# JiahaoPlus/EvoWorld

Measured on AMD Instinct MI355X. Metric: panoramic frames/sec per clip (576x1024x25f, 25 denoise steps), higher is better.
Workload: dtype f16

## Files before the change

evoworld_amd/csrc/norm.hip:

```cpp
#include "common.h"
#include <cstdlib>

namespace {

inline int gn_chunks(int n_slabs, int rows) {
    constexpr int target = 640;
    int want = (target + n_slabs - 1) / n_slabs;
    const int cap = (rows + 63) / 64;
    if (want > cap) want = cap;
    if (want > 512) want = 512;
    return want < 1 ? 1 : want;
}

__global__ void gn_stats_kernel(const f16* __restrict__ x, const int8_t* __restrict__ x_lo, float* __restrict__ part,
                                float* __restrict__ pivot, int rows, int C_src, int c_off, int C_tot, int VPP, int PL,
                                int rows_per_block) {
    extern __shared__ float lds[];
    const int tid = threadIdx.x;
    const int slab = blockIdx.y;
    const int v = tid % VPP, pl = tid / VPP;
    const int r0 = blockIdx.x * rows_per_block;
    const int r1 = min(rows, r0 + rows_per_block);
    float s[8], q[8], piv[8];
    const size_t slab_off = ((size_t)slab * rows) * C_src + v * 8;
// ... 60 lines not shown
                const float f = (float)val[e] - piv[e];
                s[e] += f;
                q[e] += f * f;
            }
        }
    }
    float* mine = lds + (size_t)pl * 2 * C_src;
#pragma unroll
    for (int e = 0; e < 8; ++e) {
        mine[v * 8 + e] = s[e];
        mine[C_src + v * 8 + e] = q[e];
    }
    __syncthreads();
    float* dst = part + (((size_t)slab * gridDim.x + blockIdx.x) * C_tot + c_off) * 2;
    for (int c = tid; c < C_src; c += blockDim.x) {
        float ss = 0.f, qq = 0.f;
        for (int k = 0; k < PL; ++k) { ss += lds[(size_t)k * 2 * C_src + c]; qq += lds[(size_t)k * 2 * C_src + C_src + c]; }
        *(f32x2*)(dst + 2 * c) = (f32x2){ss, qq};
    }
    if (blockIdx.x == 0 && pl == 0) {
#pragma unroll
        for (int e = 0; e < 8; ++e) pivot[(size_t)slab * C_tot + c_off + v * 8 + e] = piv[e];
    }
}

__global__ __launch_bounds__(256) void gn_finalize_kernel(const float* __restrict__ part, const float* __restrict__ pivot,
                                                          float* __restrict__ stats, int n_slabs, int rows, int C_tot,
                                                          int groups, int chunks) {
    __shared__ float red[2][256];
    __shared__ float chan[2][512];
    __shared__ float wsum[4];
    const int tid = threadIdx.x;
    const int slab = blockIdx.x / groups, g = blockIdx.x - slab * groups;
    const int gs = C_tot / groups;
    const float n = (float)rows;
    const int cw = gs < 256 ? gs : 256;
    const int KP = 256 / cw;
    for (int c0 = 0; c0 < gs; c0 += cw) {
        const int c = c0 + tid % cw, kc = tid / cw;
        float ss = 0.f, qq = 0.f;
        if (kc < KP && c < gs) {
            const float* p = part + (((size_t)slab * chunks) * C_tot + g * gs + c) * 2;
            for (int k = kc; k < chunks; k += KP) {
                const f32x2 v = *(const f32x2*)(p + (size_t)k * C_tot * 2);
                ss += v[0];
                qq += v[1];
            }
        }
        red[0][tid] = ss;
        red[1][tid] = qq;
        __syncthreads();
        if (tid < cw && c0 + tid < gs) {
            float s2 = 0.f, q2 = 0.f;
            for (int k = 0; k < KP; ++k) { s2 += red[0][k * cw + tid]; q2 += red[1][k * cw + tid]; }
            const float d = s2 / n;
            chan[0][c0 + tid] = pivot[(size_t)slab * C_tot + g * gs + c0 + tid] + d;
            chan[1][c0 + tid] = fmaxf(q2 - s2 * d, 0.f);
        }
        __syncthreads();
    }
    float ms = 0.f, m2 = 0.f;
    for (int c = tid; c < gs; c += 256) { ms += chan[0][c]; m2 += chan[1][c]; }
    ms = wave_sum(ms);
    m2 = wave_sum(m2);
    if ((tid & 63) == 0) wsum[tid >> 6] = ms;
    __syncthreads();
    const float mean = (wsum[0] + wsum[1] + wsum[2] + wsum[3]) / (float)gs;
    __syncthreads();
    float dev = 0.f;
    for (int c = tid; c < gs; c += 256) { const float d = chan[0][c] - mean; dev += d * d; }
    dev = wave_sum(dev);
    if ((tid & 63) == 0) { wsum[tid >> 6] = m2 + n * dev; }
    __syncthreads();
    if (tid == 0) *(f32x2*)(stats + (size_t)blockIdx.x * 2) = (f32x2){mean, (wsum[0] + wsum[1] + wsum[2] + wsum[3]) / (n * (float)gs)};
}

template <bool LO, bool YLO>
__global__ void gn_apply_kernel(const f16* __restrict__ x, const int8_t* __restrict__ x_lo, const float* __restrict__ stats,
                                const f16* __restrict__ gamma, const f16* __restrict__ beta, f16* __restrict__ y,
                                f16* __restrict__ y_lo, int ld_y, int rows,
                                int C_src, int c_off, int C_tot, int groups, float eps, int silu, int VPP, int PL,
                                int rows_per_block) {
    const int tid = threadIdx.x;
    const int slab = blockIdx.y;
    const int v = tid % VPP, pl = tid / VPP;
    const int c = v * 8;
    const int gs = C_tot / groups;
    const f16x8 gm = *(const f16x8*)(gamma + c_off + c);
    const f16x8 bt = *(const f16x8*)(beta + c_off + c);
    float scale[8], shift[8];
    int gprev = -1;
    float mean = 0.f, rstd = 0.f;
#pragma unroll
    for (int e = 0; e < 8; ++e) {
        const int g = (c_off + c + e) / gs;
        if (g != gprev) {
            gprev = g;
            const f32x2 st = *(const f32x2*)(stats + ((size_t)slab * groups + g) * 2);
            mean = st[0];
            rstd = rsqrtf(st[1] + eps);
        }
        scale[e] = rstd;
        shift[e] = mean;
    }
    const int r0 = blockIdx.x * rows_per_block;
    const int r1 = min(rows, r0 + rows_per_block);
    const f16* xin = x + ((size_t)slab * rows) * C_src + c;
    const int8_t* xlo = LO ? x_lo + ((size_t)slab * rows) * C_src + c : nullptr;
    f16* yout = y + ((size_t)slab * rows) * ld_y + c_off + c;
    f16* ylo = YLO ? y_lo + ((size_t)slab * rows) * ld_y + c_off + c : nullptr;
    int r = r0 + pl;
    for (; r + 3 * PL < r1; r += 4 * PL) {
        f16x8 val[4];
        u32x2 vlo[4];
#pragma unroll
        for (int u = 0; u < 4; ++u) {
            val[u] = *(const f16x8*)(xin + (size_t)(r + u * PL) * C_src);
            if constexpr (LO) vlo[u] = *(const u32x2*)(xlo + (size_t)(r + u * PL) * C_src);
        }
#pragma unroll
        for (int u = 0; u < 4; ++u) {
            f16x8 o, ol;
#pragma unroll
            for (int e = 0; e < 8; ++e) {
                float xv;
                if constexpr (LO) xv = ew_split_dec(val[u][e], ew_sbyte(vlo[u][e >> 2], e & 3));
                else xv = (float)val[u][e];
                float f = (xv - shift[e]) * scale[e] * (float)gm[e] + (float)bt[e];
                if (silu) f = ew_silu(f);
                o[e] = (f16)f;
                if constexpr (YLO) ol[e] = (f16)(f - (float)o[e]);
            }
            *(f16x8*)(yout + (size_t)(r + u * PL) * ld_y) = o;
            if constexpr (YLO) *(f16x8*)(ylo + (size_t)(r + u * PL) * ld_y) = ol;
        }
    }
    for (; r < r1; r += PL) {
        const f16x8 val = *(const f16x8*)(xin + (size_t)r * C_src);
        u32x2 vlo;
        if constexpr (LO) vlo = *(const u32x2*)(xlo + (size_t)r * C_src);
        f16x8 o, ol;
#pragma unroll
        for (int e = 0; e < 8; ++e) {
            float xv;
            if constexpr (LO) xv = ew_split_dec(val[e], ew_sbyte(vlo[e >> 2], e & 3));
            else xv = (float)val[e];
            float f = (xv - shift[e]) * scale[e] * (float)gm[e] + (float)bt[e];
            if (silu) f = ew_silu(f);
            o[e] = (f16)f;
            if constexpr (YLO) ol[e] = (f16)(f - (float)o[e]);
        }
        *(f16x8*)(yout + (size_t)r * ld_y) = o;
        if constexpr (YLO) *(f16x8*)(ylo + (size_t)r * ld_y) = ol;
    }
}

template <int NV, int RPW>
__global__ __launch_bounds__(256) void ln_kernel(const f16* __restrict__ x, const int8_t* __restrict__ x_lo,
                                                 const f16* __restrict__ addvec, int rpg, f16* __restrict__ x_out,
                                                 int8_t* __restrict__ x_out_lo, const f16* __restrict__ gamma,
                                                 const f16* __restrict__ beta, f16* __restrict__ y, int rows, int C,
                                                 float eps) {
    const int lane = threadIdx.x & 63;
    const int row0 = (blockIdx.x * 4 + (threadIdx.x >> 6)) * RPW;
    if (row0 >= rows) return;
    const int VPP = C / 8;
    float v[RPW][NV][8];
    f16x8 raw[RPW][NV], add[RPW][NV];
    u32x2 rlo[RPW][NV];
#pragma unroll
    for (int r = 0; r < RPW; ++r) {
        const int row = min(row0 + r, rows - 1);
#pragma unroll
        for (int k = 0; k < NV; ++k) {
            const int vi = lane + k * 64;
            if (vi < VPP) {
                raw[r][k] = *(const f16x8*)(x + (size_t)row * C + vi * 8);
                if (x_lo) rlo[r][k] = *(const u32x2*)(x_lo + (size_t)row * C + vi * 8);
                if (addvec) add[r][k] = *(const f16x8*)(addvec + (size_t)(row / rpg) * C + vi * 8);
            }
        }
    }
    f16x8 g[NV], bta[NV];
#pragma unroll
    for (int k = 0; k < NV; ++k) {
        const int vi = lane + k * 64;
        if (vi < VPP) { g[k] = *(const f16x8*)(gamma + vi * 8); bta[k] = *(const f16x8*)(beta + vi * 8); }
    }
#pragma unroll
    for (int r = 0; r < RPW; ++r) {
        const int row = row0 + r;
        const bool live = row < rows;
        float sum = 0.f;
#pragma unroll
        for (int k = 0; k < NV; ++k) {
            const int vi = lane + k * 64;
            if (vi < VPP) {
                if (x_lo) {
                    ew_split_dec8(raw[r][k], rlo[r][k], v[r][k]);
                } else {
#pragma unroll
                    for (int e = 0; e < 8; ++e) v[r][k][e] = (float)raw[r][k][e];
                }
                if (addvec) {
                    f16x8 xo;
                    int s8[8];
#pragma unroll
                    for (int e = 0; e < 8; ++e) {
                        const float sum = v[r][k][e] + (float)add[r][k][e];
                        xo[e] = (f16)sum;
                        s8[e] = ew_split_enc(sum, xo[e]);
                        v[r][k][e] = !x_out ? sum : (x_out_lo ? ew_split_dec(xo[e], s8[e]) : (float)xo[e]);
                    }
                    if (x_out && live) *(f16x8*)(x_out + (size_t)row * C + vi * 8) = xo;
                    if (x_out_lo && live)
                        *(u32x2*)(x_out_lo + (size_t)row * C + vi * 8) =
                            (u32x2){ew_pack4(s8[0], s8[1], s8[2], s8[3]), ew_pack4(s8[4], s8[5], s8[6], s8[7])};
                }
#pragma unroll
                for (int e = 0; e < 8; ++e) sum += v[r][k][e];
            } else {
#pragma unroll
                for (int e = 0; e < 8; ++e) v[r][k][e] = 0.f;
            }
        }
        const float mean = wave_sum(sum) / (float)C;
        float sq = 0.f;
#pragma unroll
        for (int k = 0; k < NV; ++k) {
            const int vi = lane + k * 64;
            if (vi < VPP) {
#pragma unroll
                for (int e = 0; e < 8; ++e) { const float d = v[r][k][e] - mean; sq += d * d; }
            }
        }
        const float rstd = rsqrtf(wave_sum(sq) / (float)C + eps);
#pragma unroll
        for (int k = 0; k < NV; ++k) {
            const int vi = lane + k * 64;
            if (vi < VPP && live) {
                f16x8 o;
#pragma unroll
                for (int e = 0; e < 8; ++e) o[e] = (f16)((v[r][k][e] - mean) * rstd * (float)g[k][e] + (float)bta[k][e]);
                *(f16x8*)(y + (size_t)row * C + vi * 8) = o;
            }
        }
    }
}

}

extern "C" size_t ew_groupnorm_workspace_floats(int n_slabs, int rows, int C_tot, int groups) {
    if (n_slabs <= 0 || rows <= 0 || C_tot <= 0 || groups <= 0) return 0;
    return (size_t)n_slabs * gn_chunks(n_slabs, rows) * C_tot * 2 + (size_t)n_slabs * C_tot + (size_t)n_slabs * groups * 2;
}

namespace {
struct GnWs { float* part; float* pivot; float* stats; int chunks; };
inline GnWs gn_ws(float* ws, int n_slabs, int rows, int C_tot) {
    GnWs w;
    w.chunks = gn_chunks(n_slabs, rows);
    w.part = ws;
    w.pivot = ws + (size_t)n_slabs * w.chunks * C_tot * 2;
    w.stats = w.pivot + (size_t)n_slabs * C_tot;
    return w;
}
}

extern "C" ew_status ew_groupnorm_stats_f16(const void* x, const void* x_lo, float* ws, int n_slabs, int rows, int C_src,
                                            int c_off, int C_tot, int groups, void* stream) {
    EW_REQUIRE(x && ws, "ew_groupnorm_stats_f16: null pointer");
    EW_REQUIRE(n_slabs > 0 && rows > 0 && C_src > 0 && C_src % 8 == 0 && C_src <= 8192, "ew_groupnorm_stats_f16: bad shape");
    EW_REQUIRE(groups > 0 && C_tot % groups == 0 && c_off >= 0 && c_off + C_src <= C_tot, "ew_groupnorm_stats_f16: bad groups");
    const int VPP = C_src / 8;
    EW_REQUIRE(VPP <= 1024, "ew_groupnorm_stats_f16: C_src too large");
    const int PL = VPP >= 256 ? 1 : 256 / VPP;
    const GnWs w = gn_ws(ws, n_slabs, rows, C_tot);
    const int rpb = ew_cdiv(rows, w.chunks);
    dim3 grid(w.chunks, n_slabs);
    const size_t lds = (size_t)PL * 2 * C_src * sizeof(float);
    EW_REQUIRE(lds <= 64 * 1024, "ew_groupnorm_stats_f16: C_src too large for the LDS combine");
    hipLaunchKernelGGL(gn_stats_kernel, grid, dim3(VPP * PL), lds, (hipStream_t)stream, (const f16*)x, (const int8_t*)x_lo,
                       w.part, w.pivot, rows, C_src, c_off, C_tot, VPP, PL, rpb);
    return ew_check_launch("ew_groupnorm_stats_f16");
}

extern "C" ew_status ew_groupnorm_finalize(float* ws, int n_slabs, int rows, int C_tot, int groups, void* stream) {
    EW_REQUIRE(ws, "ew_groupnorm_finalize: null pointer");
    EW_REQUIRE(n_slabs > 0 && rows > 0 && groups > 0 && C_tot % groups == 0 && C_tot / groups <= 512,
               "ew_groupnorm_finalize: bad shape");
    const GnWs w = gn_ws(ws, n_slabs, rows, C_tot);
    hipLaunchKernelGGL(gn_finalize_kernel, dim3(n_slabs * groups), dim3(256), 0, (hipStream_t)stream,
                       w.part, w.pivot, w.stats, n_slabs, rows, C_tot, groups, w.chunks);
    return ew_check_launch("ew_groupnorm_finalize");
}

static ew_status gn_apply_launch(const char* what, const void* x, const void* x_lo, const float* ws, const void* gamma,
                                 const void* beta, void* y, void* y_lo, int ld_y, int n_slabs, int rows, int C_src, int c_off,
                                 int C_tot, int groups, float eps, int silu, void* stream) {
    EW_REQUIRE(x && ws && gamma && beta && y, "ew_groupnorm_apply: null pointer");
    EW_REQUIRE(n_slabs > 0 && rows > 0 && C_src > 0 && C_src % 8 == 0 && c_off % 8 == 0 && C_tot % 8 == 0,
               "ew_groupnorm_apply: bad shape");
    EW_REQUIRE(groups > 0 && C_tot % groups == 0 && c_off >= 0 && c_off + C_src <= C_tot, "ew_groupnorm_apply: bad groups");
    EW_REQUIRE(ld_y >= C_tot && ld_y % 8 == 0, "ew_groupnorm_apply: bad output row stride");
    const int VPP = C_src / 8;
    EW_REQUIRE(VPP <= 1024, "ew_groupnorm_apply: C_src too large");
    const int PL = VPP >= 256 ? 1 : 256 / VPP;
    const int rpb = 8 * PL;
    const GnWs w = gn_ws((float*)ws, n_slabs, rows, C_tot);
    dim3 grid(ew_cdiv(rows, rpb), n_slabs);
#define GN_APPLY(LO_, YLO_)                                                                                                      \
    hipLaunchKernelGGL((gn_apply_kernel<LO_, YLO_>), grid, dim3(VPP * PL), 0, (hipStream_t)stream, (const f16*)x,                  \
                       (const int8_t*)x_lo, w.stats, (const f16*)gamma, (const f16*)beta, (f16*)y, (f16*)y_lo, ld_y, rows, C_src,  \
                       c_off, C_tot, groups, eps, silu, VPP, PL, rpb)
    if (x_lo) { if (y_lo) GN_APPLY(true, true); else GN_APPLY(true, false); }
    else      { if (y_lo) GN_APPLY(false, true); else GN_APPLY(false, false); }
#undef GN_APPLY
    return ew_check_launch(what);
}

extern "C" ew_status ew_groupnorm_apply_f16(const void* x, const void* x_lo, const float* ws, const void* gamma,
                                            const void* beta, void* y, int n_slabs, int rows, int C_src, int c_off, int C_tot,
                                            int groups, float eps, int silu, void* stream) {
    return gn_apply_launch("ew_groupnorm_apply_f16", x, x_lo, ws, gamma, beta, y, nullptr, C_tot, n_slabs, rows, C_src, c_off, C_tot,
                           groups, eps, silu, stream);
}

extern "C" ew_status ew_groupnorm_apply_split_f16(const void* x, const void* x_lo, const float* ws, const void* gamma,
                                                  const void* beta, void* y, void* y_lo, int ld_y, int n_slabs, int rows, int C_src,
                                                  int c_off, int C_tot, int groups, float eps, int silu, void* stream) {
    EW_REQUIRE(y_lo, "ew_groupnorm_apply_split_f16: null pointer");
    return gn_apply_launch("ew_groupnorm_apply_split_f16", x, x_lo, ws, gamma, beta, y, y_lo, ld_y, n_slabs, rows, C_src, c_off, C_tot,
                           groups, eps, silu, stream);
}

extern "C" ew_status ew_layernorm_f16(const void* x, const void* x_lo, const void* addvec, int rows_per_group, void* x_out,
                                      void* x_out_lo, const void* gamma, const void* beta, void* y, int rows, int C, float eps,
                                      void* stream) {
    EW_REQUIRE(x && gamma && beta && y, "ew_layernorm_f16: null pointer");
    EW_REQUIRE(rows > 0 && C > 0 && C % 8 == 0 && C <= 2048, "ew_layernorm_f16: need C %% 8 == 0 and C <= 2048 (C=%d)", C);
    EW_REQUIRE(!addvec || rows_per_group >= 1, "ew_layernorm_f16: rows_per_group must be >= 1");
    EW_REQUIRE(!x_out_lo || (addvec && x_out), "ew_layernorm_f16: x_out_lo needs addvec and x_out");
    const int nv = (C / 8 + 63) / 64;
    dim3 block(256);
    hipStream_t s = (hipStream_t)stream;
    const int rpg = rows_per_group >= 1 ? rows_per_group : 1;
#define LN_LAUNCH(NV, RPW)                                                                                         \
    hipLaunchKernelGGL((ln_kernel<NV, RPW>), dim3(ew_cdiv(rows, 4 * RPW)), block, 0, s, (const f16*)x, (const int8_t*)x_lo, \
                       (const f16*)addvec, rpg, (f16*)x_out, (int8_t*)x_out_lo, (const f16*)gamma, (const f16*)beta, (f16*)y, rows, C, eps)
    if (nv == 1) LN_LAUNCH(1, 4);
    else if (nv == 2) LN_LAUNCH(2, 4);
    else if (nv == 3) LN_LAUNCH(3, 2);
    else LN_LAUNCH(4, 2);
#undef LN_LAUNCH
    return ew_check_launch("ew_layernorm_f16");
}
```

evoworld_amd/ops.py:

```python
import ctypes

import numpy as np
import torch

from . import _lib
from ._lib import GemmArgs

A_DENSE, A_CONV3X3, A_CONVT3 = _lib.EW_A_DENSE, _lib.EW_A_CONV3X3, _lib.EW_A_CONVT3
ACT_NONE, ACT_SILU, ACT_GEGLU, ACT_GELU = _lib.EW_ACT_NONE, _lib.EW_ACT_SILU, _lib.EW_ACT_GEGLU, _lib.EW_ACT_GELU

_zero_pages = {}


def _stream():
    return ctypes.c_void_p(torch.cuda.current_stream().cuda_stream)


def _ptr(t):
    return None if t is None else ctypes.c_void_p(t.data_ptr())


def _call(name, *args):
    _lib.check(getattr(_lib.load(), name)(*args, _stream()), name)


def _aligned(t, n=16):
    t = t.contiguous()
    return t if t.data_ptr() % n == 0 else t.clone(memory_format=torch.contiguous_format)


def _req(t, dtype, name):
    if t.device.type != "cuda":
        raise _lib.EvoWorldHipError(f"{name} must live on the GPU (got {t.device}); evoworld_amd has no CPU path")
    if t.dtype != dtype:
        raise TypeError(f"{name}: expected {dtype}, got {t.dtype}")
    if not t.is_contiguous():
        raise ValueError(f"{name} must be contiguous")
    return t


def zero_page(device):
    key = str(device)
    if key not in _zero_pages:
        _zero_pages[key] = torch.zeros(4096, dtype=torch.float16, device=device)
    return _zero_pages[key]


class Res:
    __slots__ = ("hi", "lo")

    def __init__(self, hi, lo=None):
        self.hi, self.lo = hi, lo

    @classmethod
    def empty(cls, rows, C, device, split):
        hi = torch.empty(rows, C, dtype=torch.float16, device=device)
        return cls(hi, torch.empty(rows, C, dtype=torch.int8, device=device) if split else None)

    @classmethod
    def from_float(cls, x):
        x = x.float().contiguous()
        hi = x.half()
        d = (x.view(torch.int32) - hi.float().view(torch.int32) + 16) >> 5
        return cls(hi, d.clamp_(-128, 127).to(torch.int8))

    def float(self):
        if self.lo is None:
            return self.hi.float()
        return (self.hi.float().contiguous().view(torch.int32) + (self.lo.to(torch.int32) << 5)).view(torch.float32)


def _hl(x):
    if x is None:
        return None, None
    if isinstance(x, Res):
        return x.hi, x.lo
    return x, None


def gemm(a, w, out, *, M, N, c1, lda, a2=None, c2=0, lda2=0, bias=None, rowbias=None, rows_per_group=1, ld_rowbias=None,
         r1=None, ld_r1=0, r2=None, ld_r2=0, ld_out=None, mode=A_DENSE, conv=None, tconv=None, act=ACT_NONE,
         c_acc=1.0, c_r1=1.0, c_r2=1.0, conv_shift=0):
    g = GemmArgs()
    r1h, r1l = _hl(r1)
    r2h, r2l = _hl(r2)
    outh, outl = _hl(out)
    g.a, g.a2, g.w, g.bias, g.rowbias = _ptr(a), _ptr(a2), _ptr(w), _ptr(bias), _ptr(rowbias)
    g.r1, g.r2, g.out, g.zero_page = _ptr(r1h), _ptr(r2h), _ptr(outh), _ptr(zero_page(a.device))
    g.r1_lo, g.r2_lo, g.out_lo = _ptr(r1l), _ptr(r2l), _ptr(outl)
    g.M, g.N, g.c1, g.c2, g.lda, g.lda2 = M, N, c1, c2, lda, lda2
    n_out = N // 2 if act == ACT_GEGLU else N
    g.ld_out = ld_out if ld_out is not None else n_out
    g.ld_r1, g.ld_r2, g.mode = ld_r1, ld_r2, mode
    g.ld_rowbias = ld_rowbias if ld_rowbias is not None else N
    if conv is not None:
        g.n_img, g.h_in, g.w_in, g.h_out, g.w_out, g.stride, g.upsample = conv
    if tconv is not None:
        g.tB, g.tT, g.tP = tconv
    g.rows_per_group, g.act = rows_per_group, act
    g.c_acc, g.c_r1, g.c_r2 = c_acc, c_r1, c_r2
    g.conv_shift = conv_shift
    _call("ew_gemm_f16", ctypes.byref(g))
    return out


_sk_ready = set()


def streamk_init():
    key = (torch.cuda.current_device(), torch.cuda.current_stream().cuda_stream)
    if key in _sk_ready:
        return
    if _lib.load().ew_get_gemm_generation() != 3:
        return
    if torch.cuda.is_current_stream_capturing():
        return
    _sk_ready.add(key)
    if _lib.load().ew_gemm_streamk_init(_stream()) != 0:
        import warnings
        msg = _lib.load().ew_last_error()
        warnings.warn("ew_gemm_streamk_init: " + (msg.decode() if msg else "failed") + " (continuing without the stream-K tail on this stream)")


def streamk_check():
    st = _lib.load().ew_gemm_streamk_status()
    if st != 0:
        msg = _lib.load().ew_last_error()
        raise _lib.EvoWorldHipError((msg.decode() if msg else "stream-K hand-over timed out in ew_gemm_f16 (generation 3): results of that launch are invalid")
                                    if st > 0 else "ew_gemm_streamk_status: HIP error while reading the status word")


def linear(x, w, bias=None, out=None, split_out=False, **kw):
    _req(x, torch.float16, "x"); _req(w, torch.float16, "w")
    M, K = x.shape
    N = w.shape[0]
    act = kw.get("act", ACT_NONE)
    if out is None:
        n_out = N // 2 if act == ACT_GEGLU else N
        out = Res.empty(M, n_out, x.device, True) if split_out else torch.empty(M, n_out, dtype=torch.float16, device=x.device)
    return gemm(x, w, out, M=M, N=N, c1=K, lda=K, bias=bias, **kw)


class WorkspacePool:

    def __init__(self, device, floats=8 << 20):
        self.buf = torch.empty(floats, dtype=torch.float32, device=device)
        self.cur = 0

    def reset(self):
        self.cur = 0

    def take(self, n):
        n = (n + 63) // 64 * 64
        if self.cur + n > self.buf.numel():
            return torch.empty(n, dtype=torch.float32, device=self.buf.device)
        v = self.buf[self.cur: self.cur + n]
        self.cur += n
        return v


def groupnorm(xs, gamma, beta, n_slabs, rows, eps, silu, groups=32, out=None, pool=None, stats_hi_only=False, split_out=False):
    lib = _lib.load()
    srcs = [_hl(x) for x in xs]
    C_tot = sum(h.shape[-1] for h, _ in srcs)
    dev = srcs[0][0].device
    nws = lib.ew_groupnorm_workspace_floats(n_slabs, rows, C_tot, groups)
    ws = pool.take(nws) if pool is not None else torch.empty(nws, dtype=torch.float32, device=dev)
    if out is None:
        out = torch.empty(n_slabs * rows, 2 * C_tot if split_out else C_tot, dtype=torch.float16, device=dev)
    off = 0
    for h, l in srcs:
        _call("ew_groupnorm_stats_f16", _ptr(h), None if stats_hi_only else _ptr(l), _ptr(ws), n_slabs, rows, h.shape[-1], off, C_tot, groups)
        off += h.shape[-1]
    _call("ew_groupnorm_finalize", _ptr(ws), n_slabs, rows, C_tot, groups)
    off = 0
    for h, l in srcs:
        if split_out:
            _call("ew_groupnorm_apply_split_f16", _ptr(h), _ptr(l), _ptr(ws), _ptr(gamma), _ptr(beta), _ptr(out), _ptr(out[:, C_tot:]),
                  2 * C_tot, n_slabs, rows, h.shape[-1], off, C_tot, groups, eps, 1 if silu else 0)
        else:
            _call("ew_groupnorm_apply_f16", _ptr(h), _ptr(l), _ptr(ws), _ptr(gamma), _ptr(beta), _ptr(out), n_slabs, rows,
                  h.shape[-1], off, C_tot, groups, eps, 1 if silu else 0)
        off += h.shape[-1]
    return out


def layernorm(x, gamma, beta, eps=1e-5, addvec=None, rows_per_group=1, x_out=None, out=None):
    xh, xl = _hl(x)
    oh, ol = _hl(x_out)
    rows, C = xh.shape
    if out is None:
        out = torch.empty_like(xh)
    _call("ew_layernorm_f16", _ptr(xh), _ptr(xl), _ptr(addvec), rows_per_group, _ptr(oh), _ptr(ol), _ptr(gamma), _ptr(beta), _ptr(out), rows, C, eps)
    return out


def attn_spatial(q, k, vt, o, n_seq, S, heads, ld_qk, ld_vt, ld_o, scale=0.125):
    _call("ew_attn_spatial_f16", _ptr(q), _ptr(k), _ptr(vt), _ptr(o), n_seq, S, heads, ld_qk, ld_vt, ld_o, scale)
    return o


QK_LOG2_PRESCALE = (0.125 * 1.4426950408889634) ** 0.5


def attn_spatial_log2(q, k, vt, o, n_seq, S, heads, ld_qk, ld_vt, ld_o):
    _call("ew_attn_spatial_log2_f16", _ptr(q), _ptr(k), _ptr(vt), _ptr(o), n_seq, S, heads, ld_qk, ld_vt, ld_o)
    return o


def quant_rows_fp8(x):
    _req(x, torch.float16, "x")
    if x.ndim != 2:
        raise ValueError(f"x: expected fp16 [rows, K], got {tuple(x.shape)}")
    rows, K = x.shape
    q = torch.empty(rows, K, dtype=torch.uint8, device=x.device)
    scale = torch.empty(rows, dtype=torch.float32, device=x.device)
    _call("ew_quant_rows_fp8", _ptr(x), _ptr(q), _ptr(scale), rows, K)
    return q, scale


def gemm_fp8(aq, a_scale, wq, w_scale, out=None, c_acc=1.0):
    _req(aq, torch.uint8, "aq"); _req(wq, torch.uint8, "wq"); _req(a_scale, torch.float32, "a_scale"); _req(w_scale, torch.float32, "w_scale")
    if aq.ndim != 2 or wq.ndim != 2 or aq.shape[1] != wq.shape[1]:
        raise ValueError(f"aq {tuple(aq.shape)} / wq {tuple(wq.shape)}: expected [M, K] and [N, K]")
    M, K = aq.shape
    N = wq.shape[0]
    if a_scale.numel() != M or w_scale.numel() != N:
        raise ValueError(f"a_scale / w_scale hold {a_scale.numel()} / {w_scale.numel()} values for M, N = {M}, {N}")
    if out is None:
        out = torch.empty(M, N, dtype=torch.float16, device=aq.device)
    if out.dtype != torch.float16 or out.device != aq.device or tuple(out.shape) != (M, N) or out.stride(1) != 1:
        raise ValueError(f"out: expected an fp16 [{M}, {N}] device tensor with unit column stride, got {out.dtype} {tuple(out.shape)} strides {out.stride()}")
    _call("ew_gemm_fp8", _ptr(aq), _ptr(a_scale), _ptr(wq), _ptr(w_scale), _ptr(out), M, N, K, out.stride(0), float(c_acc))
    return out


def attn_temporal(q, k, v, o, B, T, S, heads, ld, ld_o, scale=0.125):
    _call("ew_attn_temporal_f16", _ptr(q), _ptr(k), _ptr(v), _ptr(o), B, T, S, heads, ld, ld_o, scale)
    return o


def softmax_rows(scores, out=None):
    h, l = _hl(scores)
    R, C = h.shape
    if out is None:
        out = torch.empty_like(h)
    _call("ew_softmax_rows_f16", _ptr(h), _ptr(l), _ptr(out), R, C, C)
    return out


def time_conv3(x, w, bias):
    _req(x, torch.float32, "x"); _req(w, torch.float32, "w"); _req(bias, torch.float32, "bias")
    B, T, C, H, W = x.shape
    y = torch.empty_like(x)
    _call("ew_time_conv3_f32", _ptr(x), _ptr(w), _ptr(bias), _ptr(y), B, T, C, H * W)
    return y


def sinusoid_embed(vals, n_rows, dim):
    _req(vals, torch.float32, "vals")
    out = torch.empty(n_rows, dim, dtype=torch.float16, device=vals.device)
    _call("ew_sinusoid_embed_f16", _ptr(vals), vals.numel(), n_rows, dim, _ptr(out))
    return out


def nchw_f32_to_nhwc_f16(x, y, ldc, c_off=0, scale=1.0, split=None):
    _req(x, torch.float32, "x"); _req(y, torch.float16, "y")
    N, C, H, W = x.shape
    if split:
        _call("ew_nchw_f32_to_nhwc_split_f16", _ptr(x), _ptr(y), N, C, H, W, ldc, c_off, split[0], split[1], scale)
        return y
    _call("ew_nchw_f32_to_nhwc_f16", _ptr(x), _ptr(y), N, C, H, W, ldc, c_off, scale)
    return y


def nhwc_f16_to_nchw_f32(x, N, C, H, W, ldc):
    _req(x, torch.float16, "x")
    y = torch.empty(N, C, H, W, dtype=torch.float32, device=x.device)
    _call("ew_nhwc_f16_to_nchw_f32", _ptr(x), _ptr(y), N, C, H, W, ldc)
    return y


def euler_cfg_step(eps, ld_eps, latents, guidance, sigma, sigma_next, next_in, cpad, T, h, w, split=None):
    _req(latents, torch.float32, "latents"); _req(guidance, torch.float32, "guidance")
    if split:
        _call("ew_euler_cfg_step_split", _ptr(eps), ld_eps, _ptr(latents), _ptr(guidance), float(sigma), float(sigma_next),
              _ptr(next_in), cpad, split[0], split[1], T, h, w)
        return
    _call("ew_euler_cfg_step", _ptr(eps), ld_eps, _ptr(latents), _ptr(guidance), float(sigma), float(sigma_next), _ptr(next_in), cpad, T, h, w)


def plucker_embed(rays, c2w):
    _req(rays, torch.float32, "rays"); _req(c2w, torch.float32, "c2w")
    H, W, _ = rays.shape
    N = c2w.shape[0]
    out = torch.empty(N, 6, H, W, dtype=torch.float32, device=rays.device)
    _call("ew_plucker_embed", _ptr(rays), _ptr(c2w), _ptr(out), N, H, W)
    return out


def cube2equi_gather(faces, lut, H, W):
    _req(faces, torch.uint8, "faces"); _req(lut, torch.int16, "lut")
    V, res, ch = faces.shape[0], faces.shape[2], faces.shape[-1]
    pano = torch.empty(V, H, W, 3, dtype=torch.uint8, device=faces.device)
    _call("ew_cube2equi_gather", _ptr(faces), ch, _ptr(lut), _ptr(pano), V, H, W, res)
    return pano


def equi2cube(panos, interpolation=True, out=None):
    _req(panos, torch.uint8, "panos")
    if panos.ndim != 4 or panos.shape[3] != 3:
        raise ValueError(f"panos: expected uint8 [V,H,W,3], got {tuple(panos.shape)}")
    V, H, W, _ = panos.shape
    if out is None:
        out = torch.empty(V, 3 * (W // 4), W, 3, dtype=torch.uint8, device=panos.device)
    _req(out, torch.uint8, "out")
    if tuple(out.shape) != (V, 3 * (W // 4), W, 3):
        raise ValueError(f"out: expected {(V, 3 * (W // 4), W, 3)}, got {tuple(out.shape)}")
# ... 569 lines not shown
```

include/evoworld_hip.h:

```cpp
#ifndef EVOWORLD_HIP_H
#define EVOWORLD_HIP_H
#include <stddef.h>
#include <stdint.h>
#ifdef __cplusplus
extern "C" {
#endif

typedef int ew_status;
#define EW_OK 0
#define EW_ERR_INVALID_ARG (-1)
#define EW_ERR_UNSUPPORTED (-2)
#define EW_ERR_HIP (-3)

#define EW_ABI_VERSION 19
int ew_abi_version(void);
const char* ew_last_error(void);

enum { EW_A_DENSE = 0, EW_A_CONV3X3 = 1, EW_A_CONVT3 = 2 };
enum { EW_ACT_NONE = 0, EW_ACT_SILU = 1, EW_ACT_GEGLU = 2, EW_ACT_GELU = 3  };

typedef struct ew_gemm_args {
    const void* a;
    const void* a2;
    const void* w;
    const void* bias;
    const void* rowbias;
    const void* r1;
    const void* r2;
    void* out;
    const void* zero_page;
    int M, N;
    int c1, c2;
    int lda, lda2;
    int ld_out, ld_r1, ld_r2, ld_rowbias;
    int mode;
    int n_img, h_in, w_in, h_out, w_out, stride, upsample;
    int tB, tT, tP;
    int rows_per_group;
    int act;
    float c_acc, c_r1, c_r2;
    const void* r1_lo;
    const void* r2_lo;
    void* out_lo;
    int conv_shift;
} ew_gemm_args;

ew_status ew_gemm_f16(const ew_gemm_args* args, void* stream);
void ew_set_gemm_generation(int gen);
int ew_get_gemm_generation(void);
const char* ew_gemm_last_kernel(void);
void ew_set_gemm_debug(int flags);
int ew_gemm_streamk_status(void);
ew_status ew_gemm_streamk_init(void* stream);

int ew_set_cu_budget(int n_cus);
int ew_get_cu_budget(void);
void* ew_stream_create_cu_mask(int first_cu, int n_cus);
ew_status ew_stream_destroy(void* stream);

typedef struct ew_ff_args {
    const void* x;
    const void* w1p;
    const void* b1p;
    const void* w2p;
    const void* b2;
    const void* rowbias;
    const void* r1;
    const void* r1_lo;
    const void* r2;
    const void* r2_lo;
    void* out;
    void* out_lo;
    const void* zero_page;
    int M, C, hidden;
    int rows_per_group, ld_rowbias;
    float c_acc, c_r1, c_r2;
} ew_ff_args;
ew_status ew_ff_geglu320_f16(const ew_ff_args* args, void* stream);

size_t ew_groupnorm_workspace_floats(int n_slabs, int rows, int C_tot, int groups);
ew_status ew_groupnorm_stats_f16(const void* x, const void* x_lo, float* ws, int n_slabs, int rows, int C_src, int c_off,
                                 int C_tot, int groups, void* stream);
ew_status ew_groupnorm_finalize(float* ws, int n_slabs, int rows, int C_tot, int groups, void* stream);
ew_status ew_groupnorm_apply_f16(const void* x, const void* x_lo, const float* ws, const void* gamma, const void* beta,
                                 void* y, int n_slabs, int rows, int C_src, int c_off, int C_tot, int groups, float eps,
                                 int silu, void* stream);
ew_status ew_groupnorm_apply_split_f16(const void* x, const void* x_lo, const float* ws, const void* gamma, const void* beta,
                                       void* y, void* y_lo, int ld_y, int n_slabs, int rows, int C_src, int c_off, int C_tot,
                                       int groups, float eps, int silu, void* stream);

ew_status ew_layernorm_f16(const void* x, const void* x_lo, const void* addvec, int rows_per_group, void* x_out,
                           void* x_out_lo, const void* gamma, const void* beta, void* y, int rows, int C, float eps,
                           void* stream);

ew_status ew_attn_spatial_f16(const void* q, const void* k, const void* vt, void* o, int n_seq, int S, int heads,
                              int ld_qk, long long ld_vt, int ld_o, float scale, void* stream);

ew_status ew_attn_spatial_log2_f16(const void* q, const void* k, const void* vt, void* o, int n_seq, int S, int heads,
                                   int ld_qk, long long ld_vt, int ld_o, void* stream);

ew_status ew_attn_temporal_f16(const void* q, const void* k, const void* v, void* o, int B, int T, int S, int heads,
                               int ld, int ld_o, float scale, void* stream);

ew_status ew_nchw_f32_to_nhwc_f16(const float* x, void* y, int N, int C, int H, int W, int ldc, int c_off, float scale,
                                  void* stream);
ew_status ew_nhwc_f16_to_nchw_f32(const void* x, float* y, int N, int C, int H, int W, int ldc, void* stream);
ew_status ew_nchw_f32_to_nhwc_split_f16(const float* x, void* y, int N, int C, int H, int W, int ldc, int c_off, int lo_off,
                                        int dup_off, float scale, void* stream);

ew_status ew_sinusoid_embed_f16(const float* vals, int n_vals, int n_rows, int dim, void* out, void* stream);

ew_status ew_euler_cfg_step(const void* eps, int ld_eps, float* latents, const float* guidance, float sigma,
                            float sigma_next, void* next_in, int cpad, int T, int h, int w, void* stream);
ew_status ew_euler_cfg_step_split(const void* eps, int ld_eps, float* latents, const float* guidance, float sigma,
                                  float sigma_next, void* next_in, int cpad, int lo_off, int dup_off, int T, int h, int w,
                                  void* stream);

ew_status ew_softmax_rows_f16(const void* hi, const void* lo, void* out, long long rows, int cols, long long ld, void* stream);

ew_status ew_time_conv3_f32(const float* x, const float* w, const float* bias, float* y, int B, int T, int C, int HW, void* stream);

ew_status ew_blur_axis_f32(const float* x, const float* kern, int ksize, float* out, long long planes, int H, int W, int axis,
                           void* stream);
ew_status ew_bicubic_resize_f32(const float* x, float* out, int N, int C, int H, int W, int Ho, int Wo, const float* scale,
                                const float* shift, void* stream);
ew_status ew_vit_patchify_f16(const float* x, void* out, int N, int S, int P, int ldk, void* stream);
ew_status ew_attn_small_f16(const void* q, const void* k, const void* v, void* o, int n_seq, int S, int heads, int D, int ld,
                            int ld_o, float scale, void* stream);

ew_status ew_quant_rows_fp8(const void* x, void* q, float* scale, int rows, int K, void* stream);
ew_status ew_gemm_fp8(const void* a, const float* a_scale, const void* w, const float* w_scale, void* out, int M, int N, int K,
                      long long ld_out, float c_acc, void* stream);

ew_status ew_plucker_embed(const float* rays, const float* c2w, float* out, int N, int H, int W, void* stream);

ew_status ew_cube2equi_gather(const uint8_t* faces, int face_channels, const int16_t* lut, uint8_t* pano, int V, int H,
                              int W, int res, void* stream);

ew_status ew_depth_unproject(const float* depth, const float* extr, const float* intr, float* xyz, int S, int H, int W,
                             void* stream);

size_t ew_select_workspace_bytes(void);
ew_status ew_select_kth_f32(const float* x, size_t n, size_t k, void* ws, float* out2, void* stream);
size_t ew_filter_compact_workspace_bytes(size_t n);
ew_status ew_filter_compact(const float* conf, size_t n, float thr, const float* xyz, const float* img, int img_nchw,
                            unsigned hw, float* out_xyz, unsigned* out_rgbx, void* ws, unsigned* total, void* stream);

ew_status ew_splat_cubemap(const float* xyz, size_t npts, const float* w2c, unsigned long long* zbuf, int V, int res,
                           float fx, float fy, float cx, float cy, float z_near, void* stream);
ew_status ew_splat_resolve(const unsigned long long* zbuf, const uint8_t* rgb, int rgb_stride, uint8_t* faces,
                           int face_channels, int V, int res, void* stream);

size_t ew_points_bounds_workspace_bytes(size_t n);
ew_status ew_points_bounds(const float* xyz, size_t n, void* ws, float* out6, unsigned long long* n_finite, void* stream);
ew_status ew_voxel_keys(const float* xyz, size_t n, const float* origin3, float voxel, long long* keys, int* overflow, void* stream);
size_t ew_voxel_reduce_workspace_bytes(size_t n);
ew_status ew_voxel_reduce(const long long* sorted_keys, const long long* perm, size_t n, const float* xyz, const uint8_t* rgbx,
                          float* out_xyz, uint8_t* out_rgba, int* out_count, void* ws, unsigned long long* n_voxels, void* stream);

#define EW_JPEG_420 420
#define EW_JPEG_444 444
size_t ew_jpeg_segment_slot_bytes(int mcu_cols, int blocks_per_mcu);
ew_status ew_jpeg_dct_quant(const uint8_t* frames, int16_t* coef, int V, int H, int W, int quality, int subsampling, void* stream);
ew_status ew_jpeg_entropy(const int16_t* coef, uint8_t* slots, int* seg_bytes, long long n_segments, int mcu_cols, int blocks_per_mcu,
                          size_t slot_bytes, void* stream);
ew_status ew_jpeg_pack(const uint8_t* slots, const int* seg_bytes, const long long* seg_offsets, uint8_t* out, long long n_segments,
                       int mcu_rows, size_t slot_bytes, long long out_bytes, void* stream);

ew_status ew_equi2pers(const uint8_t* equi, const float* rot, uint8_t* out, int F, int He, int We, int Hp, int Wp,
                       float fov_x_deg, void* stream);

ew_status ew_resize_aa_u8(const uint8_t* src, uint8_t* tmp, uint8_t* dst, const int* kk_h, const int* bounds_h, int ksize_h,
                          const int* kk_v, const int* bounds_v, int ksize_v, int V, int Hi, int Wi, int Ho, int Wo, void* stream);
ew_status ew_u8_hwc_to_f32_chw(const uint8_t* src, float* dst, int V, int H, int W, void* stream);
ew_status ew_f32_chw_to_u8_hwc(const float* src, uint8_t* dst, int V, int H, int W, void* stream);

ew_status ew_pano_yaw_rotate(const void* src, int src_u8, const float* yaw_deg, float* dst, int V, int H, int W, void* stream);

size_t ew_video_metrics_workspace_bytes(int F, int C, int H, int W);
ew_status ew_video_metrics(const void* a, const void* b, int layout, int F, int C, int H, int W, int what, double* sse, double* ssim,
                           void* workspace, void* stream);

size_t ew_video_metrics_ws_workspace_bytes(int F, int C, int H, int W);
ew_status ew_video_metrics_ws(const void* a, const void* b, int layout, int F, int C, int H, int W, int what, const double* row_w,
                              double* wsse, double* wssim, void* workspace, void* stream);

ew_status ew_gt_dump_map_u8(const uint8_t* src, uint8_t* dst, size_t n, void* stream);

ew_status ew_equi2cube_u8(const uint8_t* pano, uint8_t* cross, int V, int H, int W, int interpolation, void* stream);

enum { EW_IM2COL_F16_NHWC = 0, EW_IM2COL_U8_HWC = 1, EW_IM2COL_F32_CHW = 2 };
ew_status ew_im2col_f16(const void* src, int src_kind, void* out, int n_img, int h_in, int w_in, int C, int k, int stride, int pad,
                        int h_out, int w_out, int ldk, int relu, int swap_rb, const float* first_affine, void* stream);
ew_status ew_maxpool3s2_relu_f16(const void* src, void* out, int n_img, int h_in, int w_in, int C, int h_out, int w_out, void* stream);
size_t ew_lpips_head_workspace_bytes(int F, int h, int w, int C);
ew_status ew_lpips_head(const void* fa, const void* fb, const float* lin, const double* wy, const double* wx, int F, int h, int w, int C,
                        double n_out, double* acc, void* workspace, void* stream);

ew_status ew_video_preprocess_f16(const void* src, int src_kind, void* out, int T, int H, int W, int h_resized, int w_resized, int y0, int x0,
                                  int swap_rb, void* stream);
ew_status ew_im2col3d_f16(const void* src, void* out, int t_in, int h_in, int w_in, int C, int kt, int kh, int kw, int st, int sh, int sw,
                          int pt, int ph, int pw, int t_out, int h_out, int w_out, int ldk, int relu, void* stream);
ew_status ew_maxpool3d_relu_f16(const void* src, void* out, int t_in, int h_in, int w_in, int C, int kt, int kh, int kw, int st, int sh, int sw,
                                int pt, int ph, int pw, int t_out, int h_out, int w_out, void* stream);
size_t ew_i3d_head_workspace_bytes(void);
ew_status ew_i3d_head(const void* x, int t_in, int h_in, int w_in, int C, const float* w, const float* b, float* logits, void* workspace,
                      void* stream);

ew_status ew_frames_resize_aa_norm_f16(const void* src, int src_kind, void* out, int F, int H, int W, int out_h, int out_w, const int* y_first,
                                       const int* y_count, const float* y_weights, int y_taps, const int* x_first, const int* x_count,
                                       const float* x_weights, int x_taps, int swap_rb, const float* mean_std, void* stream);
ew_status ew_avgpool3x3_relu_f16(const void* src, void* out, int n_img, int H, int W, int C, void* stream);
ew_status ew_global_avgpool_relu_f32(const void* src, float* out, int n_img, int h, int w, int C, void* stream);

#ifdef __cplusplus
}
#endif
#endif
```

Measured before the change: 5.284.

## Add single-pass fused GroupNorm kernel holding each group in registers

Adds a GroupNorm kernel where one workgroup owns a (slab, group) pair. It loads that group's values into registers once, computes the mean and a two-pass variance with block reductions, then applies the affine transform and optional SiLU, with optional split hi/lo output. This replaces the separate stats, finalize and apply launches and the second read of the input, when the group fits within the register budget. It also adds an XCD-aware workgroup index remap. It risks low occupancy from high register use, and few workgroups when n_slabs*groups is small.

```diff
diff --git a/evoworld_amd/csrc/norm.hip b/evoworld_amd/csrc/norm.hip
--- a/evoworld_amd/csrc/norm.hip
+++ b/evoworld_amd/csrc/norm.hip
@@ -236,6 +236,153 @@
         }
         *(f16x8*)(yout + (size_t)r * ld_y) = o;
         if constexpr (YLO) *(f16x8*)(ylo + (size_t)r * ld_y) = ol;
+    }
+}
+
+constexpr int GN_FUSED_MAX_NK = 12;
+constexpr int GN_FUSED_MAX_NT = 1024;
+constexpr int GN_FUSED_MAX_GS = 512;
+#define GN_FUSED_WAVES 8
+
+template <int U> struct GnUnit;
+template <> struct GnUnit<4> { typedef f16x4 hi_t; typedef unsigned lo_t; };
+template <> struct GnUnit<2> { typedef f16x2 hi_t; typedef unsigned short lo_t; };
+
+struct GnFusedArgs {
+    const f16* x0; const int8_t* x0_lo; const f16* x1; const int8_t* x1_lo;
+    const f16* gamma; const f16* beta; f16* y; f16* y_lo;
+    int C0, C1, ld_y, rows, groups, gs, silu, remap;
+    float eps;
+};
+
+__device__ __forceinline__ float gn_block_sum(float v, float* red) {
+    v = wave_sum(v);
+    if ((threadIdx.x & 63) == 0) red[threadIdx.x >> 6] = v;
+    __syncthreads();
+    float t = 0.f;
+    const int nw = blockDim.x >> 6;
+    for (int w = 0; w < nw; ++w) t += red[w];
+    __syncthreads();
+    return t;
+}
+
+template <int U, int NK, bool LO, bool TWO>
+__global__ __launch_bounds__(GN_FUSED_MAX_NT) __attribute__((amdgpu_waves_per_eu(GN_FUSED_WAVES))) void gn_fused_kernel(const GnFusedArgs a) {
+    typedef typename GnUnit<U>::hi_t hi_t;
+    typedef typename GnUnit<U>::lo_t lo_t;
+    __shared__ __attribute__((aligned(16))) f16 sg[GN_FUSED_MAX_GS];
+    __shared__ __attribute__((aligned(16))) f16 sb[GN_FUSED_MAX_GS];
+    __shared__ float red[GN_FUSED_MAX_NT / 64];
+    const int tid = threadIdx.x, NT = blockDim.x;
+    int bid = blockIdx.x;
+    if (a.remap) {
+        const int nwg = gridDim.x;
+        const int qq = nwg >> 3, r = nwg & 7, xcd = bid & 7, idx = bid >> 3;
+        bid = (xcd < r ? xcd * (qq + 1) : r * (qq + 1) + (xcd - r) * qq) + idx;
+    }
+    const int slab = bid / a.groups, g = bid - slab * a.groups;
+    const int gs = a.gs, upr = gs / U, c0 = g * gs;
+    const int n_units = a.rows * upr;
+    for (int i = tid; i < gs; i += NT) { sg[i] = a.gamma[c0 + i]; sb[i] = a.beta[c0 + i]; }
+    const int dq = NT / upr, dr = NT - dq * upr;
+    const int row0 = tid / upr, u0 = tid - row0 * upr;
+    const size_t s0 = (size_t)slab * a.rows * a.C0, s1 = (size_t)slab * a.rows * a.C1;
+    const f16* const b0 = a.x0 + s0;
+    const f16* const b1 = TWO ? a.x1 + s1 : b0;
+    const bool h0 = a.x0_lo != nullptr, h1 = TWO && a.x1_lo != nullptr;
+    const int8_t* const l0 = h0 ? a.x0_lo + s0 : (const int8_t*)b0;
+    const int8_t* const l1 = h1 ? a.x1_lo + s1 : (const int8_t*)b1;
+
+    hi_t hi[NK];
+    lo_t lo[NK];
+    {
+        int row = row0, u = u0;
+#pragma unroll
+        for (int k = 0; k < NK; ++k) {
+            const bool live = tid + k * NT < n_units;
+            const int rr = live ? row : 0, c = c0 + (live ? u : 0) * U;
+            const bool first = !TWO || c < a.C0;
+            const int off = first ? rr * a.C0 + c : rr * a.C1 + (c - a.C0);
+            hi[k] = *(const hi_t*)((first ? b0 : b1) + off);
+            lo[k] = 0;
+            if constexpr (LO) {
+                const lo_t v = *(const lo_t*)((first ? l0 : l1) + off);
+                lo[k] = (first ? h0 : h1) ? v : (lo_t)0;
+            }
+            u += dr; row += dq;
+            if (u >= upr) { u -= upr; ++row; }
+        }
+    }
+#pragma unroll
+    for (int k = 0; k < NK; ++k)
+        if (!(tid + k * NT < n_units)) { hi[k] = (hi_t)(f16)0.f; lo[k] = 0; }
+    auto value2 = [&](int k, int e) -> f32x2 {
+        if constexpr (LO) return (f32x2){ew_split_dec(hi[k][e], ew_sbyte((unsigned)lo[k], e)), ew_split_dec(hi[k][e + 1], ew_sbyte((unsigned)lo[k], e + 1))};
+        else return (f32x2){(float)hi[k][e], (float)hi[k][e + 1]};
+    };
+    auto redecode = [&]() {
+#pragma unroll
+        for (int k = 0; k < NK; ++k) {
+            asm volatile("" : "+v"(hi[k]));
+            if constexpr (LO) asm volatile("" : "+v"(lo[k]));
+        }
+    };
+    const float n = (float)a.rows * (float)gs;
+    f32x2 s2 = {0.f, 0.f};
+#pragma unroll
+    for (int k = 0; k < NK; ++k)
+#pragma unroll
+        for (int e = 0; e < U; e += 2) s2 += value2(k, e);
+    const float mean = gn_block_sum(s2[0] + s2[1], red) / n;
+    const f32x2 mean2 = {mean, mean};
+    redecode();
+    f32x2 q2 = {0.f, 0.f};
+#pragma unroll
+    for (int k = 0; k < NK; ++k) {
+        if (tid + k * NT < n_units) {
+#pragma unroll
+            for (int e = 0; e < U; e += 2) { const f32x2 d = value2(k, e) - mean2; q2 = __builtin_elementwise_fma(d, d, q2); }
+        }
+    }
+    const float rstd = rsqrtf(gn_block_sum(q2[0] + q2[1], red) / n + a.eps);
+    const f32x2 rstd2 = {rstd, rstd};
+    redecode();
+
+    f16* const yb = a.y + (size_t)slab * a.rows * a.ld_y + c0;
+    f16* const ylb = a.y_lo ? a.y_lo + (size_t)slab * a.rows * a.ld_y + c0 : nullptr;
+    {
+        int row = row0, u = u0;
+        asm volatile("" : "+v"(row), "+v"(u));
+#pragma unroll
+        for (int k = 0; k < NK; ++k) {
+            if (tid + k * NT < n_units) {
+                const hi_t gm = *(const hi_t*)(sg + u * U), bt = *(const hi_t*)(sb + u * U);
+                float f[U];
+#pragma unroll
+                for (int e = 0; e < U; e += 2) {
+                    const f32x2 t = (value2(k, e) - mean2) * rstd2;
+                    const f32x2 r = __builtin_elementwise_fma(t, (f32x2){(float)gm[e], (float)gm[e + 1]}, (f32x2){(float)bt[e], (float)bt[e + 1]});
+                    f[e] = r[0]; f[e + 1] = r[1];
+                }
+                if (a.silu) {
+#pragma unroll
+                    for (int e = 0; e < U; ++e) f[e] = f[e] * __builtin_amdgcn_rcpf(1.0f + __expf(-f[e]));
+                }
+                hi_t o;
+#pragma unroll
+                for (int e = 0; e < U; ++e) o[e] = (f16)f[e];
+                const int off = row * a.ld_y + u * U;
+                *(hi_t*)(yb + off) = o;
+                if (ylb) {
+                    hi_t ol;
+#pragma unroll
+                    for (int e = 0; e < U; ++e) ol[e] = (f16)(f[e] - (float)o[e]);
+                    *(hi_t*)(ylb + off) = ol;
+                }
+            }
+            u += dr; row += dq;
+            if (u >= upr) { u -= upr; ++row; }
+        }
     }
 }
 
@@ -418,6 +565,86 @@
                            groups, eps, silu, stream);
 }
 
+namespace {
+struct GnFusedPlan { int U, units, NT, NK; };
+int g_gn_fused_nt = 0;
+int g_gn_fused_remap = 1;
+
+inline bool gn_fused_plan(int rows, int C_tot, int groups, int n_src, int nt_force, GnFusedPlan& p) {
+    if (rows <= 0 || C_tot <= 0 || groups <= 0 || C_tot % groups != 0 || C_tot % 8 != 0) return false;
+    if (n_src < 1 || n_src > 2) return false;
+    const int gs = C_tot / groups;
+    if (gs % 2 != 0 || gs > GN_FUSED_MAX_GS) return false;
+    p.U = gs % 4 == 0 ? 4 : 2;
+    const long long units = (long long)rows * (gs / p.U);
+    if (units > (long long)GN_FUSED_MAX_NT * GN_FUSED_MAX_NK) return false;
+    p.units = (int)units;
+    int nt = nt_force ? nt_force : (p.units <= 256 * 12 ? 256 : p.units <= 512 * 12 ? 512 : 1024);
+    while (nt < GN_FUSED_MAX_NT && (long long)nt * GN_FUSED_MAX_NK < units) nt *= 2;
+    p.NT = nt;
+    const int per = ew_cdiv(p.units, nt);
+    p.NK = per <= 4 ? 4 : 12;
+    return true;
+}
+}
+
+extern "C" int ew_groupnorm_fused_ok(int rows, int C_tot, int groups, int n_src) {
+    GnFusedPlan p;
+    return gn_fused_plan(rows, C_tot, groups, n_src, 0, p) ? 1 : 0;
+}
+
+extern "C" int ew_groupnorm_fused_preferred(int n_slabs, int rows, int C_tot, int groups, int n_src) {
+    GnFusedPlan p;
+    if (n_slabs <= 0 || !gn_fused_plan(rows, C_tot, groups, n_src, 0, p)) return 0;
+    return C_tot / groups >= 40 || p.NT == 256;
+}
+
+extern "C" ew_status ew_groupnorm_fused_set_tuning(int threads, int remap) {
+    EW_REQUIRE(threads == 0 || threads == 256 || threads == 512 || threads == 1024, "ew_groupnorm_fused_set_tuning: threads must be 0 (automatic), 256, 512 or 1024");
+    g_gn_fused_nt = threads;
+    g_gn_fused_remap = remap ? 1 : 0;
+    return EW_OK;
+}
+
+extern "C" ew_status ew_groupnorm_fused_f16(const void* x0, const void* x0_lo, int C0, const void* x1, const void* x1_lo, int C1,
+                                            const void* gamma, const void* beta, void* y, void* y_lo, int ld_y, int n_slabs, int rows,
+                                            int groups, float eps, int silu, void* stream) {
+    EW_REQUIRE(x0 && gamma && beta && y, "ew_groupnorm_fused_f16: null pointer");
+    EW_REQUIRE(n_slabs > 0 && rows > 0 && C0 > 0 && C0 % 8 == 0 && C1 >= 0 && C1 % 8 == 0, "ew_groupnorm_fused_f16: bad shape");
+    EW_REQUIRE((C1 == 0) == (x1 == nullptr) && (x1 || !x1_lo), "ew_groupnorm_fused_f16: second source and C1 must come together");
+    const long long C_tot = (long long)C0 + C1;
+    EW_REQUIRE(groups > 0 && C_tot % groups == 0, "ew_groupnorm_fused_f16: bad groups");
+    EW_REQUIRE(ld_y >= C_tot && ld_y % 8 == 0, "ew_groupnorm_fused_f16: bad output row stride");
+    EW_REQUIRE(((uintptr_t)x0 | (uintptr_t)x1 | (uintptr_t)y | (uintptr_t)y_lo) % 8 == 0 && ((uintptr_t)x0_lo | (uintptr_t)x1_lo) % 4 == 0,
+               "ew_groupnorm_fused_f16: unaligned pointer");
+    EW_REQUIRE((long long)rows * ld_y < (1LL << 31) && (long long)n_slabs * groups < (1LL << 31), "ew_groupnorm_fused_f16: slab too large for 32-bit offsets");
+    GnFusedPlan p;
+    if (C_tot > (1 << 20) || !gn_fused_plan(rows, (int)C_tot, groups, x1 ? 2 : 1, g_gn_fused_nt, p)) {
+        ew_set_error("ew_groupnorm_fused_f16: a (slab, group) of rows=%d x %lld channels does not fit one workgroup (ew_groupnorm_fused_ok)", rows,
+                     C_tot / groups);
+        return EW_ERR_UNSUPPORTED;
+    }
+    GnFusedArgs a;
+    a.x0 = (const f16*)x0; a.x0_lo = (const int8_t*)x0_lo; a.x1 = (const f16*)x1; a.x1_lo = (const int8_t*)x1_lo;
+    a.gamma = (const f16*)gamma; a.beta = (const f16*)beta; a.y = (f16*)y; a.y_lo = (f16*)y_lo;
+    a.C0 = C0; a.C1 = C1; a.ld_y = ld_y; a.rows = rows; a.groups = groups; a.gs = (int)C_tot / groups; a.silu = silu;
+    a.remap = g_gn_fused_remap; a.eps = eps;
+    const dim3 grid(n_slabs * groups), block(p.NT);
+    const bool lo = x0_lo || x1_lo;
+#define GN_FUSED(U_, NK_)                                                                                             \
+    do {                                                                                                              \
+        if (lo && x1) hipLaunchKernelGGL((gn_fused_kernel<U_, NK_, true, true>), grid, block, 0, (hipStream_t)stream, a);    \
+        else if (lo) hipLaunchKernelGGL((gn_fused_kernel<U_, NK_, true, false>), grid, block, 0, (hipStream_t)stream, a);    \
+        else if (x1) hipLaunchKernelGGL((gn_fused_kernel<U_, NK_, false, true>), grid, block, 0, (hipStream_t)stream, a);    \
+        else hipLaunchKernelGGL((gn_fused_kernel<U_, NK_, false, false>), grid, block, 0, (hipStream_t)stream, a);           \
+    } while (0)
+    static_assert(GN_FUSED_MAX_NK == 12, "the instantiations below");
+    if (p.U == 4) { if (p.NK == 4) GN_FUSED(4, 4); else GN_FUSED(4, 12); }
+    else          { if (p.NK == 4) GN_FUSED(2, 4); else GN_FUSED(2, 12); }
+#undef GN_FUSED
+    return ew_check_launch("ew_groupnorm_fused_f16");
+}
+
 extern "C" ew_status ew_layernorm_f16(const void* x, const void* x_lo, const void* addvec, int rows_per_group, void* x_out,
                                       void* x_out_lo, const void* gamma, const void* beta, void* y, int rows, int C, float eps,
                                       void* stream) {
diff --git a/evoworld_amd/ops.py b/evoworld_amd/ops.py
--- a/evoworld_amd/ops.py
+++ b/evoworld_amd/ops.py
@@ -1,4 +1,5 @@
 import ctypes
+import os
 
 import numpy as np
 import torch
@@ -10,6 +11,7 @@
 ACT_NONE, ACT_SILU, ACT_GEGLU, ACT_GELU = _lib.EW_ACT_NONE, _lib.EW_ACT_SILU, _lib.EW_ACT_GEGLU, _lib.EW_ACT_GELU
 
 _zero_pages = {}
+GN_FUSED = os.environ.get("EW_GN_FUSED", "1") != "0"
 
 
 def _stream():
@@ -164,6 +166,14 @@
     srcs = [_hl(x) for x in xs]
     C_tot = sum(h.shape[-1] for h, _ in srcs)
     dev = srcs[0][0].device
+    if GN_FUSED and not stats_hi_only and len(srcs) <= 2 and lib.ew_groupnorm_fused_preferred(n_slabs, rows, C_tot, groups, len(srcs)):
+        if out is None:
+            out = torch.empty(n_slabs * rows, 2 * C_tot if split_out else C_tot, dtype=torch.float16, device=dev)
+        (h0, l0), (h1, l1) = srcs[0], (srcs[1] if len(srcs) == 2 else (None, None))
+        _call("ew_groupnorm_fused_f16", _ptr(h0), _ptr(l0), h0.shape[-1], _ptr(h1), _ptr(l1), 0 if h1 is None else h1.shape[-1], _ptr(gamma),
+              _ptr(beta), _ptr(out), _ptr(out[:, C_tot:]) if split_out else None, 2 * C_tot if split_out else C_tot, n_slabs, rows, groups, eps,
+              1 if silu else 0)
+        return out
     nws = lib.ew_groupnorm_workspace_floats(n_slabs, rows, C_tot, groups)
     ws = pool.take(nws) if pool is not None else torch.empty(nws, dtype=torch.float32, device=dev)
     if out is None:
diff --git a/include/evoworld_hip.h b/include/evoworld_hip.h
--- a/include/evoworld_hip.h
+++ b/include/evoworld_hip.h
@@ -88,6 +88,12 @@
 ew_status ew_groupnorm_apply_split_f16(const void* x, const void* x_lo, const float* ws, const void* gamma, const void* beta,
                                        void* y, void* y_lo, int ld_y, int n_slabs, int rows, int C_src, int c_off, int C_tot,
                                        int groups, float eps, int silu, void* stream);
+int ew_groupnorm_fused_ok(int rows, int C_tot, int groups, int n_src);
+int ew_groupnorm_fused_preferred(int n_slabs, int rows, int C_tot, int groups, int n_src);
+ew_status ew_groupnorm_fused_set_tuning(int threads, int remap);
+ew_status ew_groupnorm_fused_f16(const void* x0, const void* x0_lo, int C0, const void* x1, const void* x1_lo, int C1,
+                                 const void* gamma, const void* beta, void* y, void* y_lo, int ld_y, int n_slabs, int rows,
+                                 int groups, float eps, int silu, void* stream);
 
 ew_status ew_layernorm_f16(const void* x, const void* x_lo, const void* addvec, int rows_per_group, void* x_out,
                            void* x_out_lo, const void* gamma, const void* beta, void* y, int rows, int C, float eps,
```

Result: no change. 5.310, median of 6 (+0.5%).
